# tensorflow/recommenders

Hardware: NVIDIA H100
Metric: queries/sec brute-force top-K (1Mx64 candidates) (higher is better)
Workload: dtype f32 (fp16 wgmma screening, fp32 accumulate + exact fp32 re-scoring)

## Files before the change

### include/tfrs_b200.h

```cpp
#ifndef TFRS_B200_H_
#define TFRS_B200_H_

#include <stddef.h>
#include <stdint.h>

#ifdef __cplusplus
extern "C" {
#endif

#define TFRS_B200_VERSION 102

enum {
  TFRS_OK = 0,
  TFRS_ERR_INVALID_ARG = -1,
  TFRS_ERR_UNSUPPORTED = -2,
  TFRS_ERR_CUDA = -3,
  TFRS_ERR_WORKSPACE_TOO_SMALL = -4,
  TFRS_ERR_NCCL = -5
};

enum { TFRS_I32 = 0, TFRS_I64 = 1 };

int tfrs_version(void);
const char* tfrs_last_error(void);
// ... 6 lines not shown
size_t tfrs_topk_scan_workspace_bytes(int64_t Q, int64_t N, int d, int k);
int tfrs_topk_scan_f32(const float* q, int64_t Q, const float* corpus, int64_t N, int d, int k,
                       int64_t index_offset, const float* state_scores, const int64_t* state_idx,
                       int state_k, float* out_scores, int64_t* out_idx, void* ws, size_t ws_bytes,
                       void* stream);

size_t tfrs_index_bytes(int64_t N, int d);
int tfrs_index_build(const float* corpus, int64_t N, int d, void* index_buf, size_t index_bytes,
                     void* stream);
size_t tfrs_topk_tc_workspace_bytes(int64_t Q, int64_t N, int d, int k);
int tfrs_topk_tc_f32(const float* q, int64_t Q, const float* corpus, const void* index_buf, int64_t N,
                     int d, int k, int64_t index_offset, float* out_scores, int64_t* out_idx, void* ws,
                     size_t ws_bytes, void* stream);

int tfrs_topk_tc_exclude_f32(const float* q, int64_t Q, const float* corpus, const void* index_buf, int64_t N, int d,
                             int k, int64_t index_offset, const int64_t* identifiers, const int64_t* exclusions,
                             int n_excl, float* out_scores, int64_t* out_idx, void* ws, size_t ws_bytes, void* stream);

int tfrs_topk_tc_count_f32(const float* q, int64_t Q, const float* corpus, const void* index_buf, int64_t N, int d,
                           int k, const float* positive_scores, int32_t* out_count, void* ws, size_t ws_bytes,
                           void* stream);

int tfrs_topk_exclude_rerank_f32(const float* scores, const int64_t* idx, int64_t Q, int k_fetched,
                                 const int64_t* identifiers, const int64_t* exclusions, int n_excl, int k_out,
                                 float* out_scores, int64_t* out_idx, void* stream);

int tfrs_count_above_f32(const float* scores, int64_t ld, int k, const float* positive_scores, int64_t Q,
                         int32_t* out_count, void* stream);

int tfrs_topk_hits_accumulate(const int32_t* count, const float* positive_scores, const float* sample_weight, int64_t Q,
                              const int32_t* ks, int n_ks, double* acc, void* stream);

int tfrs_topk_tc_layout(int64_t Q, int64_t N, int d, int k, int64_t* out10);

int tfrs_profile_enable(int on);
int tfrs_profile_read(float* stage_ms, int* calls);

int tfrs_topk_merge_strided(const float* scores, const int64_t* idx, int64_t list_stride_scores,
                            int64_t list_stride_idx, int n_lists, int64_t Q, int k_in, int k_out,
                            float* out_scores, int64_t* out_idx, void* stream);

int tfrs_topk_merge_sorted_strided(const float* scores, const int64_t* idx, int64_t list_stride_scores,
                                   int64_t list_stride_idx, int n_lists, int64_t Q, int k_in, int k_out,
                                   float* out_scores, int64_t* out_idx, void* stream);

typedef struct tfrs_comm* tfrs_comm_t;
int tfrs_comm_unique_id(void* out128);
int tfrs_comm_create(tfrs_comm_t* comm, int rank, int world, const void* unique_id128);
int tfrs_comm_destroy(tfrs_comm_t comm);
int tfrs_comm_enable_p2p(tfrs_comm_t comm, int64_t max_Q, int max_k);
int tfrs_comm_p2p_capacity(tfrs_comm_t comm, int64_t Q, int k);
int tfrs_comm_set_option(tfrs_comm_t comm, int option, int value);
int tfrs_comm_rank(tfrs_comm_t comm);
int tfrs_comm_world(tfrs_comm_t comm);
int tfrs_topk_allgather(tfrs_comm_t comm, const float* s, const int64_t* i, int64_t Q, int k, float* all_s,
                        int64_t* all_i, void* stream);
size_t tfrs_topk_sharded_workspace_bytes(int world, int64_t Q, int64_t N_local, int d, int k);
int tfrs_topk_sharded_layout(int world, int64_t Q, int64_t N_local, int d, int k, int64_t* out4);
int tfrs_topk_sharded_f32(tfrs_comm_t comm, const float* q, int64_t Q, const float* corpus_local, const void* index_buf,
                          int64_t N_local, int d, int k, int64_t index_offset, float* out_scores, int64_t* out_idx,
                          void* ws, size_t ws_bytes, void* stream);

int tfrs_sgemm_f32(int transA, int transB, int64_t M, int64_t N, int64_t K, const float* A, int64_t lda,
                   const float* B, int64_t ldb, float* C, int64_t ldc, int accumulate, void* stream);
int tfrs_rowwise_dot_f32(const float* a, const float* b, int64_t rows, int d, float* out, void* stream);

// ... 199 lines not shown
```

### recommenders_b200/_ffi.py

```python
from __future__ import annotations

import ctypes
import os
from typing import Optional

import torch

_HERE = os.path.dirname(os.path.abspath(__file__))
LIB_PATH = os.environ.get("TFRS_B200_LIB", os.path.join(_HERE, "libtfrs_b200.so"))

_lib: Optional[ctypes.CDLL] = None

I32, I64, BYTES = 0, 1, 2
c_p = ctypes.c_void_p
c_i = ctypes.c_int
c_l = ctypes.c_int64
c_f = ctypes.c_float
c_sz = ctypes.c_size_t

_SIGNATURES = {
    "tfrs_version": (c_i, []),
    "tfrs_last_error": (ctypes.c_char_p, []),
    "tfrs_launch_count": (c_l, []),
    "tfrs_gather_f32": (c_i, [c_p, c_p, c_p, c_i, c_p, c_i, c_l, c_p, c_l, c_p, c_p]),
    "tfrs_topk_scan_workspace_bytes": (c_sz, [c_l, c_l, c_i, c_i]),
    "tfrs_topk_scan_f32": (c_i, [c_p, c_l, c_p, c_l, c_i, c_i, c_l, c_p, c_p, c_i, c_p, c_p, c_p, c_sz, c_p]),
    "tfrs_index_bytes": (c_sz, [c_l, c_i]),
    "tfrs_index_build": (c_i, [c_p, c_l, c_i, c_p, c_sz, c_p]),
    "tfrs_topk_tc_workspace_bytes": (c_sz, [c_l, c_l, c_i, c_i]),
    "tfrs_topk_tc_f32": (c_i, [c_p, c_l, c_p, c_p, c_l, c_i, c_i, c_l, c_p, c_p, c_p, c_sz, c_p]),
    "tfrs_topk_tc_exclude_f32": (c_i, [c_p, c_l, c_p, c_p, c_l, c_i, c_i, c_l, c_p, c_p, c_i, c_p, c_p, c_p, c_sz, c_p]),
    "tfrs_topk_tc_count_f32": (c_i, [c_p, c_l, c_p, c_p, c_l, c_i, c_i, c_p, c_p, c_p, c_sz, c_p]),
    "tfrs_topk_exclude_rerank_f32": (c_i, [c_p, c_p, c_l, c_i, c_p, c_p, c_i, c_i, c_p, c_p, c_p]),
    "tfrs_count_above_f32": (c_i, [c_p, c_l, c_i, c_p, c_l, c_p, c_p]),
    "tfrs_topk_hits_accumulate": (c_i, [c_p, c_p, c_p, c_l, c_p, c_i, c_p, c_p]),
    "tfrs_topk_tc_layout": (c_i, [c_l, c_l, c_i, c_i, c_p]),
    "tfrs_dot_interaction_out_dim": (c_i, [c_i, c_i, c_i]),
    "tfrs_dot_interaction_fwd_f32": (c_i, [c_p, c_l, c_i, c_i, c_i, c_i, c_p, c_p]),
    "tfrs_dot_interaction_bwd_f32": (c_i, [c_p, c_p, c_l, c_i, c_i, c_i, c_i, c_p, c_p]),
    "tfrs_profile_enable": (c_i, [c_i]),
    "tfrs_profile_read": (c_i, [c_p, c_p]),
    "tfrs_topk_merge_strided": (c_i, [c_p, c_p, c_l, c_l, c_i, c_l, c_i, c_i, c_p, c_p, c_p]),
    "tfrs_topk_merge_sorted_strided": (c_i, [c_p, c_p, c_l, c_l, c_i, c_l, c_i, c_i, c_p, c_p, c_p]),
    "tfrs_comm_unique_id": (c_i, [c_p]),
    "tfrs_comm_create": (c_i, [c_p, c_i, c_i, c_p]),
    "tfrs_comm_destroy": (c_i, [c_p]),
    "tfrs_comm_enable_p2p": (c_i, [c_p, c_l, c_i]),
    "tfrs_comm_p2p_capacity": (c_i, [c_p, c_l, c_i]),
    "tfrs_comm_set_option": (c_i, [c_p, c_i, c_i]),
    "tfrs_comm_rank": (c_i, [c_p]),
    "tfrs_comm_world": (c_i, [c_p]),
    "tfrs_topk_allgather": (c_i, [c_p, c_p, c_p, c_l, c_i, c_p, c_p, c_p]),
    "tfrs_topk_sharded_workspace_bytes": (c_sz, [c_i, c_l, c_l, c_i, c_i]),
    "tfrs_topk_sharded_layout": (c_i, [c_i, c_l, c_l, c_i, c_i, c_p]),
    "tfrs_topk_sharded_f32": (c_i, [c_p, c_p, c_l, c_p, c_p, c_l, c_i, c_i, c_l, c_p, c_p, c_p, c_sz, c_p]),
    "tfrs_sgemm_f32": (c_i, [c_i, c_i, c_l, c_l, c_l, c_p, c_l, c_p, c_l, c_p, c_l, c_i, c_p]),
    "tfrs_rowwise_dot_f32": (c_i, [c_p, c_p, c_l, c_i, c_p, c_p]),
    "tfrs_inbatch_softmax_workspace_bytes": (c_sz, [c_l, c_l, c_i]),
    "tfrs_inbatch_softmax_fwd": (c_i, [c_p, c_p, c_l, c_l, c_i, c_f, c_p, c_p, c_p, c_p, c_sz, c_p]),
    "tfrs_inbatch_softmax_bwd": (c_i, [c_p, c_p, c_l, c_l, c_i, c_f, c_p, c_p, c_p, c_p, c_p, c_p, c_sz, c_p]),
    "tfrs_inbatch_softmax_tc_workspace_bytes": (c_sz, [c_l, c_l, c_i, c_i, c_i]),
    "tfrs_inbatch_softmax_tc_fwd": (c_i, [c_p, c_p, c_l, c_l, c_i, c_f, c_p, c_p, c_p, c_p, c_p, c_p, c_p, c_sz, c_p]),
    "tfrs_inbatch_softmax_tc_bwd_workspace_bytes": (c_sz, [c_l, c_l, c_i, c_i, c_i]),
    "tfrs_inbatch_softmax_tc_bwd": (c_i, [c_p, c_p, c_l, c_l, c_i, c_f, c_p, c_p, c_p, c_p, c_p, c_p, c_p, c_p, c_p, c_sz, c_p]),
    "tfrs_inbatch_softmax_maxsim_workspace_bytes": (c_sz, [c_l, c_i, c_l, c_i]),
    "tfrs_inbatch_softmax_maxsim_fwd": (c_i, [c_p, c_p, c_l, c_i, c_l, c_i, c_f, c_p, c_p, c_p, c_p, c_sz, c_p]),
    "tfrs_inbatch_softmax_maxsim_bwd": (c_i, [c_p, c_p, c_l, c_i, c_l, c_i, c_f, c_p, c_p, c_p, c_p, c_p, c_p, c_sz, c_p]),
    "tfrs_hardneg_loss_fwd": (c_i, [c_p, c_p, c_l, c_i, c_p, c_f, c_p, c_p, c_p, c_p]),
    "tfrs_hardneg_loss_bwd": (c_i, [c_p, c_p, c_l, c_l, c_i, c_p, c_i, c_p, c_p, c_p, c_p, c_p]),
# ... 140 lines not shown
```

### recommenders_b200/csrc/topk_tc.cu

```cuda
#include <cuda_fp16.h>
#include <math.h>
#include <stdlib.h>
#include <type_traits>
#include "rowselect.cuh"
#include "tc_ptx.cuh"

namespace tfrs {
namespace tc {

constexpr int TILE_N = 128;
constexpr int TILE_M = 128;
constexpr int QBLK = 256;
constexpr int KSLAB = 64;
constexpr int SLAB_BYTES = TILE_N * 128;
constexpr int HEADER_BYTES = 1024;
constexpr int THREADS = 512;
constexpr int CONSUMER_WARPS = 16;
constexpr int CAND_CAP = 2048;
constexpr int MAX_SAMPLE_STRIDE = 4;
constexpr int FIN_MAX_PARTS = 2 * 132;
constexpr int MAX_BINS = 1024;
constexpr int FP16_TARGET = 15;
constexpr float E_REL = 0.00108f;
constexpr float E_ACC = 0.00013f;
// ... 99 lines not shown
  const long long tile = row / TILE_N;
  if (lane < kb * 8) {
    const int slab = lane >> 3, cj = lane & 7;
    const int k0 = slab * KSLAB + cj * 8;
    __align__(16) __half v[8];
#pragma unroll
    for (int j = 0; j < 8; ++j) {
      const float f = (real && k0 + j < d) ? p[k0 + j] : 0.f;
      v[j] = __float2half_rn(ldexpf(f, e));
    }
    unsigned char* dst = qimg + tile * ((long long)kb * SLAB_BYTES) + (long long)slab * SLAB_BYTES + r * 128 + ((cj ^ (r & 7)) * 16);
    *reinterpret_cast<uint4*>(dst) = *reinterpret_cast<const uint4*>(v);
  }
}

enum { MODE_SAMPLE = 0, MODE_FILTER = 1 };

enum { FILTER_FULL = 0, FILTER_NO_EMIT = 1, FILTER_NO_EPILOGUE = 2 };
#if defined(TFRS_DEBUG_SWITCHES) && defined(TFRS_FILTER_ABLATION)
constexpr int FILTER_ABLATION = TFRS_FILTER_ABLATION;
#else
constexpr int FILTER_ABLATION = FILTER_FULL;
#endif

struct ScanParams {
  const unsigned char* qimg;
  const unsigned char* cimg;
  long long Q, N;
  int nqb, parts, n_seq, stride;
  long long n_tiles;
  float* binmax; int bins_ld;
  int group, bins_per_part;
  const float* thr;
  unsigned int* count;
  float* cand_s;
  unsigned int* cand_i;
  int cap_part;
};

template <int KB, int STAGES, int MODE>
__global__ void __launch_bounds__(THREADS, 1)
tc_scan_kernel(const ScanParams p) {
  extern __shared__ __align__(1024) unsigned char smem_raw[];
  unsigned char* smem = reinterpret_cast<unsigned char*>((reinterpret_cast<uintptr_t>(smem_raw) + 1023) & ~uintptr_t(1023));
  unsigned char* sA = smem;
  unsigned char* sB = smem + 2 * KB * SLAB_BYTES;
  uint64_t* bars = reinterpret_cast<uint64_t*>(sB + STAGES * KB * SLAB_BYTES);
  uint64_t* full = bars;
  uint64_t* empty = bars + STAGES;
  uint64_t* a_full = bars + 2 * STAGES;

  const int wg = threadIdx.x >> 7, warp = (threadIdx.x >> 5) & 3, lane = threadIdx.x & 31;
  const int qb = blockIdx.x % p.nqb, part = blockIdx.x / p.nqb;
  const int u_begin = (int)((long long)part * p.n_seq / p.parts);
  const int u_end = (int)((long long)(part + 1) * p.n_seq / p.parts);
  const int n_iter = u_end - u_begin;
  const bool issuer = threadIdx.x == 0;

  if (issuer) {
    for (int s = 0; s < STAGES; ++s) { mbar_init(&full[s], 1); mbar_init(&empty[s], CONSUMER_WARPS); }
    mbar_init(a_full, 1);
    asm volatile("fence.mbarrier_init.release.cluster;" ::: "memory");
  }
  __syncthreads();

  auto load_tile = [&](int it, int stage) {
    const long long tile = (long long)(u_begin + it) * p.stride;
    mbar_expect_tx(&full[stage], KB * SLAB_BYTES);
    if (MODE == MODE_FILTER)
      bulk_g2s_hint(sB + stage * KB * SLAB_BYTES, p.cimg + tile * ((long long)KB * SLAB_BYTES), KB * SLAB_BYTES, &full[stage],
                    l2_policy_evict_first());
    else
      bulk_g2s(sB + stage * KB * SLAB_BYTES, p.cimg + tile * ((long long)KB * SLAB_BYTES), KB * SLAB_BYTES, &full[stage]);
  };
  if (issuer) {
    mbar_expect_tx(a_full, 2 * KB * SLAB_BYTES);
    bulk_g2s(sA, p.qimg + (long long)qb * 2 * KB * SLAB_BYTES, 2 * KB * SLAB_BYTES, a_full);
    for (int it = 0; it < STAGES && it < n_iter; ++it) load_tile(it, it);
  }

  const long long row_a = (long long)qb * QBLK + wg * 64 + warp * 16 + (lane >> 2);
  const bool quad_leader = (lane & 3) == 0;
  float thr[2] = {INFINITY, INFINITY};
  if (MODE == MODE_FILTER) {
#pragma unroll
    for (int rr = 0; rr < 2; ++rr) if (row_a + 8 * rr < p.Q) thr[rr] = p.thr[row_a + 8 * rr];
  }
  const unsigned int cap = (unsigned int)p.cap_part;
  unsigned int cnt[4] = {0u, 0u, 0u, 0u}, ovf = 0u;
  unsigned int sink = 0u;
  long long seg_base[2];
#pragma unroll
  for (int rr = 0; rr < 2; ++rr) seg_base[rr] = ((row_a + 8 * rr) * p.parts + part) * 2 * (long long)cap;
  float binm[4] = {-INFINITY, -INFINITY, -INFINITY, -INFINITY};
  int in_group = 0, bin_out = 0;

  mbar_wait(a_full, 0);
  const uint32_t a0 = smem_u32(sA + (wg >> 1) * KB * SLAB_BYTES + (wg & 1) * 8192);
  uint32_t afrag[4][4];
  if (KB == 1) {
    const int r = warp * 16 + ((lane >> 3) & 1) * 8 + (lane & 7);
#pragma unroll
    for (int k4 = 0; k4 < 4; ++k4) ldmatrix_x4(afrag[k4], a0 + r * 128 + (((2 * k4 + (lane >> 4)) ^ (lane & 7)) * 16));
  }
  auto issue = [&](float (&acc)[32], int stage, int h) {
    wgmma_fence();
#pragma unroll
    for (int kb = 0; kb < KB; ++kb) {
      const uint64_t b_desc = make_smem_desc(smem_u32(sB + (stage * KB + kb) * SLAB_BYTES + h * 8192));
#pragma unroll
      for (int k4 = 0; k4 < 4; ++k4) {
        if (KB == 1)
          wgmma_m64n64_rs(acc, afrag[k4], b_desc + (uint64_t)(k4 * 2), (uint32_t)(k4 != 0));
        else
          wgmma_m64n64_ss(acc, make_smem_desc(a0 + kb * SLAB_BYTES) + (uint64_t)(k4 * 2), b_desc + (uint64_t)(k4 * 2),
                          (uint32_t)((kb | k4) != 0));
      }
    }
    wgmma_commit();
// ... 92 lines not shown
    __syncwarp();
    if (lane == 0) mbar_arrive(&empty[stage]);
    if (!LAST && issuer && it >= 1 && it - 1 + STAGES < n_iter) {
      mbar_wait(&empty[prev_stage], prev_phase);
      load_tile(it - 1 + STAGES, prev_stage);
    }
    prev_stage = stage; prev_phase = phase;
    stage = next_stage; phase = next_phase;
    epilogue(acc1, col0, it, std::integral_constant<int, 1>{});
    if (!LAST) {
      wgmma_wait<0>();
      acc_fence(acc0);
    }
  };
  if (n_iter > 0) {
    mbar_wait(&full[0], 0);
    issue(acc0, 0, 0);
    wgmma_wait<0>();
    acc_fence(acc0);
    for (int it = 0; it + 1 < n_iter; ++it) tile_step(it, std::false_type{});
    tile_step(n_iter - 1, std::true_type{});
  }
  if (MODE == MODE_SAMPLE) {
#pragma unroll
    for (int s = 0; s < 4; ++s) {
      const long long row = row_a + 8 * (s >> 1);
      if (quad_leader && row < p.Q)
        for (int b = bin_out; b < p.bins_per_part; ++b)
          p.binmax[row * p.bins_ld + (long long)part * p.bins_per_part * 2 + (s & 1) + 2 * b] = -INFINITY;
    }
  } else if (quad_leader) {
#pragma unroll
    for (int s = 0; s < 4; ++s)
      p.count[((row_a + 8 * (s >> 1)) * p.parts + part) * 2 + (s & 1)] =
          FILTER_ABLATION != FILTER_FULL ? sink : ((ovf >> s) & 1u) ? (cap + 1u) : cnt[s];
  }
}

__device__ __forceinline__ unsigned int f2key(float f) {
  unsigned int u = __float_as_uint(f);
  return (u & 0x80000000u) ? ~u : (u | 0x80000000u);
}
__device__ __forceinline__ float key2f(unsigned int k) {
  return __uint_as_float((k & 0x80000000u) ? (k & 0x7fffffffu) : ~k);
}
__device__ __forceinline__ unsigned long long rank_key(float s, unsigned int idx) {
  const unsigned int lo = (0xFFFFFFFEu - 2u * idx) | (__float_as_uint(s) == 0x80000000u ? 1u : 0u);
  return ((unsigned long long)f2key(s + 0.0f) << 32) | lo;
}
__device__ __forceinline__ float rank_key_score(unsigned long long e) {
  return __uint_as_float(__float_as_uint(key2f((unsigned int)(e >> 32))) | ((unsigned int)e << 31));
}
__device__ __forceinline__ unsigned int rank_key_index(unsigned long long e) { return 0x7FFFFFFFu - ((unsigned int)e >> 1); }
__device__ __forceinline__ int warp_incl_scan(int v, int lane) {
#pragma unroll
  for (int o = 1; o < 32; o <<= 1) { const int t = __shfl_up_sync(0xffffffffu, v, o); if (lane >= o) v += t; }
  return v;
}

template <int KPL>
__device__ __forceinline__ unsigned int warp_kth_largest_regs(const unsigned int (&key)[KPL], int k, unsigned int prefix = 0, int top_bit = 31) {
  for (int bit = top_bit; bit >= 0; --bit) {
    const unsigned int cand = prefix | (1u << bit);
    int c = 0;
#pragma unroll
    for (int j = 0; j < KPL; ++j) c += (key[j] >= cand) ? 1 : 0;
    c = __reduce_add_sync(0xffffffffu, c);
    if (c >= k) prefix = cand;
  }
  return prefix;
}
__device__ __forceinline__ unsigned int warp_kth_largest_smem(const unsigned int* keys, int n, int k, int lane, unsigned int prefix, int top_bit) {
  for (int bit = top_bit; bit >= 0; --bit) {
    const unsigned int cand = prefix | (1u << bit);
    int c = 0;
    for (int t = lane; t < n; t += 32) c += (keys[t] >= cand) ? 1 : 0;
    c = __reduce_add_sync(0xffffffffu, c);
    if (c >= k) prefix = cand;
  }
  return prefix;
}

template <int KPL>
__global__ void __launch_bounds__(256)
tc_threshold_kernel(const float* __restrict__ binmax, int bins_ld, int n_bins, int k, const float* __restrict__ margin,
                    float* __restrict__ thr, unsigned int* __restrict__ overflow, long long Q) {
  const int lane = threadIdx.x & 31;
  const long long row = ((long long)blockIdx.x * 256 + threadIdx.x) >> 5;
  if (row >= Q) return;
  const float* src = binmax + row * bins_ld;
  unsigned int key[KPL];
#pragma unroll
  for (int j = 0; j < KPL; ++j) { const int i = j * 32 + lane; key[j] = i < n_bins ? f2key(__ldg(src + i)) : 0u; }
  const unsigned int kth = warp_kth_largest_regs<KPL>(key, k);
  if (lane == 0) { thr[row] = key2f(kth) - margin[row]; overflow[row] = 0; }
}

enum { FIN_TOPK = 0, FIN_EXCLUDE = 1, FIN_COUNT = 2 };
constexpr int FW_WARPS = 4;

struct FinParams {
  const float* q; const float* corpus; int d; int k; long long index_offset; long long N; long long Q;
  const unsigned int* count; const float* cand_s; const unsigned int* cand_i; int segs; int cap_part;
  const float* cut; const float* thr; unsigned int* overflow;
  int cap_keys, cap_band;
  unsigned int* band_idx; int* band_n;
  int allow_short;
  float* out_s; long long* out_i;
  const long long* identifiers; const long long* exclusions; int n_excl; int k_out;
  const float* pos; const int* qexp; const IndexHeader* hdr; int* out_count;
};

__device__ __forceinline__ float exact_score(const float* __restrict__ qs, const float* __restrict__ c, int d) {
  float acc = 0.f;
  if ((d & 31) == 0) {
    for (int kk = 0; kk < d; kk += 32) {
      float4 cv[8];
#pragma unroll
      for (int u = 0; u < 8; ++u) cv[u] = __ldg(reinterpret_cast<const float4*>(c + kk) + u);
#pragma unroll
      for (int u = 0; u < 8; ++u) {
        acc = fmaf(qs[kk + 4 * u], cv[u].x, acc); acc = fmaf(qs[kk + 4 * u + 1], cv[u].y, acc);
        acc = fmaf(qs[kk + 4 * u + 2], cv[u].z, acc); acc = fmaf(qs[kk + 4 * u + 3], cv[u].w, acc);
      }
    }
  } else if ((d & 3) == 0) {
    for (int kk = 0; kk < d; kk += 4) {
      const float4 cv = __ldg(reinterpret_cast<const float4*>(c + kk));
      acc = fmaf(qs[kk], cv.x, acc); acc = fmaf(qs[kk + 1], cv.y, acc);
      acc = fmaf(qs[kk + 2], cv.z, acc); acc = fmaf(qs[kk + 3], cv.w, acc);
    }
  } else {
    for (int kk = 0; kk < d; ++kk) acc = fmaf(qs[kk], __ldg(c + kk), acc);
  }
  return acc;
}

// ... 39 lines not shown
    for (int j = 0; j < kf; ++j) rank += (akey[j] > mine) ? 1 : 0;
    if (rank < p.k_out) {
      const unsigned long long e = srt[t];
      p.out_s[row * p.k_out + rank] = rank_key_score(e);
      p.out_i[row * p.k_out + rank] = (long long)rank_key_index(e) + p.index_offset;
    }
  }
}

__host__ __device__ inline size_t sel_warp_bytes(int cap_keys, int segs) {
  return (size_t)cap_keys * 4 + (size_t)cap_keys * 2 + (size_t)((segs + 1 + 3) & ~3) * 4;
}
constexpr int SEL_WARPS = 8;

__device__ __forceinline__ bool load_record(const FinParams& p, long long row, const int* soff, int rec, int total_rec,
                                            unsigned int& ix0, float (&sc)[8]) {
  if (rec >= total_rec) return false;
  int lo = 0, hi = p.segs;
  while (hi - lo > 1) { const int mid = (lo + hi) >> 1; if (soff[mid] <= rec) lo = mid; else hi = mid; }
  const long long at = (row * p.segs + lo) * p.cap_part + (rec - soff[lo]);
  ix0 = __ldg(p.cand_i + at);
  const float4 s0 = __ldg(reinterpret_cast<const float4*>(p.cand_s + at * 8));
  const float4 s1 = __ldg(reinterpret_cast<const float4*>(p.cand_s + at * 8) + 1);
  sc[0] = s0.x; sc[1] = s0.y; sc[2] = s0.z; sc[3] = s0.w; sc[4] = s1.x; sc[5] = s1.y; sc[6] = s1.z; sc[7] = s1.w;
  return true;
}

template <int MODE>
__global__ void __launch_bounds__(SEL_WARPS * 32)
tc_select_kernel(const FinParams p) {
  extern __shared__ __align__(16) unsigned char fsm[];
  const int warp = threadIdx.x >> 5, lane = threadIdx.x & 31;
  const long long row = (long long)blockIdx.x * SEL_WARPS + warp;
  if (row >= p.Q) return;
  unsigned char* base = fsm + (size_t)warp * sel_warp_bytes(p.cap_keys, p.segs);
  unsigned int* keys = reinterpret_cast<unsigned int*>(base);
  unsigned short* loc = reinterpret_cast<unsigned short*>(keys + p.cap_keys);
  int* soff = reinterpret_cast<int*>(loc + p.cap_keys);
  const unsigned int n32 = (unsigned int)p.N;
  unsigned int* band = p.band_idx + row * p.cap_band;

  int carry = 0; bool bad = false;
  for (int s0 = 0; s0 < p.segs; s0 += 32) {
    const int s = s0 + lane;
    int c = 0;
    if (s < p.segs) {
      const unsigned int cc = __ldg(p.count + row * p.segs + s);
      if (cc > (unsigned int)p.cap_part) bad = true; else c = (int)cc;
    }
    const int inc = warp_incl_scan(c, lane);
    if (s < p.segs) soff[s + 1] = carry + inc;
    carry += __shfl_sync(0xffffffffu, inc, 31);
  }
  if (lane == 0) soff[0] = 0;
  if (__any_sync(0xffffffffu, bad)) {
    if (lane == 0) { p.overflow[row] = 1; p.band_n[row] = 0; }
    return;
  }
  __syncwarp();
  const int total_rec = soff[p.segs];
  const float thr_row = p.thr[row];
  if (MODE != FIN_COUNT && total_rec >= 8192) {
    if (lane == 0) { p.overflow[row] = 1; p.band_n[row] = 0; }
    return;
  }

  if (MODE == FIN_COUNT) {
// ... 29 lines not shown
      else { p.out_count[row] = definite; p.band_n[row] = m; p.overflow[row] = 0; }
    }
    return;
  }

  int n = 0;
  unsigned int kmax = 0u, kmin = 0xFFFFFFFFu;
  for (int rb = 0; rb < total_rec; rb += 32) {
    float sc[8]; unsigned int ix0 = 0, keep = 0; int cnt = 0;
    if (load_record(p, row, soff, rb + lane, total_rec, ix0, sc)) {
#pragma unroll
      for (int j = 0; j < 8; ++j) {
        const bool kp = sc[j] >= thr_row && ix0 + j < n32;
        keep |= kp ? (1u << j) : 0u; cnt += kp ? 1 : 0;
      }
    }
    const int incl = warp_incl_scan(cnt, lane);
    const int tot = __shfl_sync(0xffffffffu, incl, 31);
    if (n + tot <= p.cap_keys) {
      int at_pos = n + incl - cnt;
#pragma unroll
      for (int j = 0; j < 8; ++j) {
        if (keep & (1u << j)) {
          const unsigned int key = f2key(sc[j] + 0.0f);
          kmax = max(kmax, key); kmin = min(kmin, key);
          keys[at_pos] = key;
          loc[at_pos] = (unsigned short)(((rb + lane) << 3) | j);
          ++at_pos;
        }
      }
    }
    n += tot;
  }
  if (n > p.cap_keys || (n < p.k && !p.allow_short)) { if (lane == 0) { p.overflow[row] = 1; p.band_n[row] = 0; } return; }
  __syncwarp();
  if (n < p.k) {
    const bool fits = n <= p.cap_band;
    for (int t = lane; t < n && fits; t += 32) {
      const unsigned int l = loc[t];
      const int rec = (int)(l >> 3);
      int lo = 0, hi = p.segs;
      while (hi - lo > 1) { const int mid = (lo + hi) >> 1; if (soff[mid] <= rec) lo = mid; else hi = mid; }
      band[t] = __ldg(p.cand_i + (row * p.segs + lo) * p.cap_part + (rec - soff[lo])) + (l & 7u);
    }
    if (lane == 0) { p.overflow[row] = fits ? 0u : 1u; p.band_n[row] = fits ? n : 0; }
    return;
  }
  kmax = __reduce_max_sync(0xffffffffu, kmax); kmin = __reduce_min_sync(0xffffffffu, kmin);
  unsigned int tau_key;
  {
    const unsigned int diff = kmax ^ kmin;
    const int top = diff ? (31 - __clz(diff)) : -1;
    const unsigned int prefix0 = top >= 31 ? 0u : (top < 0 ? kmax : (kmax & ~((2u << top) - 1u)));
    if (n <= 512) {
      unsigned int kr[16];
#pragma unroll
      for (int j = 0; j < 16; ++j) { const int t = j * 32 + lane; kr[j] = t < n ? keys[t] : 0u; }
      tau_key = warp_kth_largest_regs<16>(kr, p.k, prefix0, top);
    } else if (n <= 1024) {
      unsigned int kr[32];
#pragma unroll
      for (int j = 0; j < 32; ++j) { const int t = j * 32 + lane; kr[j] = t < n ? keys[t] : 0u; }
      tau_key = warp_kth_largest_regs<32>(kr, p.k, prefix0, top);
    } else {
      tau_key = warp_kth_largest_smem(keys, n, p.k, lane, prefix0, top);
    }
  }
  const float lim = key2f(tau_key) - p.cut[row];
  if (!p.allow_short && (!(lim >= thr_row) || !(lim > -INFINITY))) { if (lane == 0) { p.overflow[row] = 1; p.band_n[row] = 0; } return; }
  const unsigned int lim_key = f2key(lim + 0.0f);
  const unsigned int lt_mask = (1u << lane) - 1u;
  int m = 0;
  for (int tb = 0; tb < n; tb += 32) {
    const int t = tb + lane;
    const bool kp = t < n && keys[t] >= lim_key;
    const unsigned int vote = __ballot_sync(0xffffffffu, kp);
    if (kp) {
      const int at_pos = m + __popc(vote & lt_mask);
      if (at_pos < p.cap_band) {
        const unsigned int l = loc[t];
        const int rec = (int)(l >> 3);
        int lo = 0, hi = p.segs;
        while (hi - lo > 1) { const int mid = (lo + hi) >> 1; if (soff[mid] <= rec) lo = mid; else hi = mid; }
        band[at_pos] = __ldg(p.cand_i + (row * p.segs + lo) * p.cap_part + (rec - soff[lo])) + (l & 7u);
      }
    }
    m += __popc(vote);
  }
  if (lane == 0) {
    if (m > p.cap_band) { p.overflow[row] = 1; p.band_n[row] = 0; }
    else { p.overflow[row] = 0; p.band_n[row] = m; }
  }
}

constexpr int RS_BLOCK = 128;
template <int MODE>
__global__ void __launch_bounds__(RS_BLOCK)
tc_rescore_kernel(const FinParams p) {
  extern __shared__ __align__(16) unsigned char rsm[];
  unsigned long long* sk = reinterpret_cast<unsigned long long*>(rsm);
  float* qs = reinterpret_cast<float*>(sk + p.cap_band);
  unsigned long long* srt = reinterpret_cast<unsigned long long*>(qs + ((p.d + 3) & ~3));
// ... 124 lines not shown
  for (long long t = threadIdx.x; t < N; t += 256) {
    const float* cr = corpus + t * d;
    float acc = 0.f;
    for (int kk = 0; kk < d; ++kk) acc = fmaf(qs[kk], __ldg(cr + kk), acc);
    c += (acc + 0.0f > ps) ? 1 : 0;
  }
  c = __reduce_add_sync(0xffffffffu, c);
  if ((threadIdx.x & 31) == 0) atomicAdd(&total, c);
  __syncthreads();
  if (threadIdx.x == 0) out_count[row] = total < k ? total : k;
}

struct Prof {
  bool on = false;
  static constexpr int MAXC = 512, STAGES_ = 4;
  cudaEvent_t ev[MAXC][STAGES_ + 1];
  int created = 0, calls = 0;
};
static Prof g_prof;
static void prof_mark(cudaStream_t st, int stage) {
  if (!g_prof.on || g_prof.calls >= Prof::MAXC) return;
  int c = g_prof.calls;
  while (g_prof.created <= c) {
    for (int s = 0; s <= Prof::STAGES_; ++s) cudaEventCreate(&g_prof.ev[g_prof.created][s]);
    ++g_prof.created;
  }
  cudaEventRecord(g_prof.ev[c][stage], st);
  if (stage == Prof::STAGES_) ++g_prof.calls;
}

struct Plan {
  int kb, stages; long long n_tiles; int nqb; long long Qp;
  int stride, n_sample, group, bins_per_part, n_bins, bins_ld, parts_sample, parts_full, cap_part, cap_keys, cap_band;
  size_t smem;
  size_t o_qimg, o_margin, o_cut, o_thr, o_qexp, o_count, o_ovf, o_binmax, o_cand, o_tmp, o_band, o_bandn, total;
};

static bool make_plan(long long Q, long long N, int d, int k, Plan& pl) {
  if (d <= 0 || d > 128 || Q <= 0 || N <= 0 || k <= 0) return false;
  pl.kb = (d + KSLAB - 1) / KSLAB;
  pl.stages = pl.kb == 1 ? 6 : 4;
  pl.n_tiles = ceil_div(N, TILE_N);
  pl.nqb = (int)ceil_div(Q, QBLK);
  pl.Qp = (long long)pl.nqb * QBLK;
  if (k > 256 || N >= (1ll << 31)) return false;
  const long long full_tiles = N / TILE_N;
  if (full_tiles < 1) return false;
  pl.stride = MAX_SAMPLE_STRIDE;
#ifdef TFRS_DEBUG_SWITCHES
  { static int ov = getenv("TFRS_TC_SAMPLE_STRIDE") ? atoi(getenv("TFRS_TC_SAMPLE_STRIDE")) : 0; if (ov >= 1 && ov <= 16) pl.stride = ov; }
#endif
  while (pl.stride > 1 && 2 * ceil_div(full_tiles, pl.stride) < 4ll * k) pl.stride >>= 1;
  pl.n_sample = (int)ceil_div(full_tiles, pl.stride);
  if (2ll * pl.n_sample < 4ll * k) return false;
  const int sms = sm_count();
  int parts = sms / pl.nqb; if (parts < 1) parts = 1; if (parts > FIN_MAX_PARTS / 2) parts = FIN_MAX_PARTS / 2;
  pl.parts_sample = parts < pl.n_sample ? parts : pl.n_sample;
  pl.parts_full = (long long)parts < pl.n_tiles ? parts : (int)pl.n_tiles;
  {
    const int iters_max = (int)ceil_div(pl.n_sample, pl.parts_sample);
    const int target = 4 * k > 512 ? 4 * k : 512;
    int g = 1;
    while ((long long)pl.parts_sample * ceil_div(iters_max, g) * 2 > target && g < iters_max) ++g;
    pl.group = g;
    pl.bins_per_part = (int)ceil_div(iters_max, g);
    pl.n_bins = pl.parts_sample * pl.bins_per_part * 2;
    if (pl.n_bins > MAX_BINS || pl.n_bins < 2 * k) return false;
    pl.bins_ld = (pl.n_bins + 31) / 32 * 32;
  }
  {
    const double lambda = (double)k * pl.stride / (pl.parts_full * 2.0);
    const double want = 2.0 * lambda + 12.0 * sqrt(lambda) + 8.0;
    int p2 = 32; while (p2 < want && p2 < 512) p2 <<= 1;
    pl.cap_part = p2;
    int ck = 1024; while (ck < 1.6 * 1.3 * k * pl.stride && ck < 4096) ck <<= 1;
    pl.cap_keys = ck;
    pl.cap_band = ck / 2;
  }
  pl.smem = (size_t)(2 + pl.stages) * pl.kb * SLAB_BYTES + 1024  + 256 ;
  size_t o = 0;
  auto take = [&](size_t bytes) { size_t r = o; o += align_up(bytes, 1024); return r; };
  pl.o_qimg = take((size_t)pl.nqb * 2 * pl.kb * SLAB_BYTES);
  pl.o_margin = take((size_t)pl.Qp * 4);
  pl.o_cut = take((size_t)pl.Qp * 4);
  pl.o_thr = take((size_t)pl.Qp * 4);
  pl.o_qexp = take((size_t)pl.Qp * 4);
  pl.o_count = take((size_t)pl.Qp * pl.parts_full * 2 * 4);
  pl.o_ovf = take((size_t)pl.Qp * 4);
  pl.o_binmax = take((size_t)pl.Qp * pl.bins_ld * 4);
  pl.o_cand = take((size_t)pl.Qp * pl.parts_full * 2 * pl.cap_part * (8 * 4 + 4));
  pl.o_tmp = take((size_t)Q * k * 12);
  pl.o_band = take((size_t)pl.Qp * pl.cap_band * 4);
  pl.o_bandn = take((size_t)pl.Qp * 4);
  pl.total = o;
  return true;
}

template <int KB, int STAGES>
static int launch_scans(const Plan& pl, ScanParams sp, cudaStream_t st, int mode) {
  auto ks = tc_scan_kernel<KB, STAGES, MODE_SAMPLE>;
  auto kf = tc_scan_kernel<KB, STAGES, MODE_FILTER>;
  TFRS_DYN_SMEM(ks, (int)pl.smem);
  TFRS_DYN_SMEM(kf, (int)pl.smem);
  if (mode == MODE_SAMPLE) {
    sp.parts = pl.parts_sample; sp.n_seq = pl.n_sample; sp.stride = pl.stride;
    ks<<<(unsigned)(pl.nqb * sp.parts), THREADS, pl.smem, st>>>(sp);
  } else {
    sp.parts = pl.parts_full; sp.n_seq = (int)pl.n_tiles; sp.stride = 1;
    kf<<<(unsigned)(pl.nqb * sp.parts), THREADS, pl.smem, st>>>(sp);
  }
  TFRS_LAUNCH_CHECK();
  return TFRS_OK;
}

static int launch_scan_mode(const Plan& pl, const ScanParams& sp, cudaStream_t st, int mode) {
  if (pl.kb == 1) return launch_scans<1, 6>(pl, sp, st, mode);
  return launch_scans<2, 4>(pl, sp, st, mode);
}

template <int MODE>
static int launch_finalize(FinParams fp, cudaStream_t st) {
  auto ksel = tc_select_kernel<MODE>;
  auto krs = tc_rescore_kernel<MODE>;
  TFRS_DYN_SMEM(ksel, (int)(SEL_WARPS * sel_warp_bytes(4096, FIN_MAX_PARTS)));
  ksel<<<(unsigned)ceil_div(fp.Q, SEL_WARPS), SEL_WARPS * 32, SEL_WARPS * sel_warp_bytes(fp.cap_keys, fp.segs), st>>>(fp);
  TFRS_LAUNCH_CHECK();
  const size_t rs_smem = (size_t)fp.cap_band * 8 + (size_t)((fp.d + 3) & ~3) * 4 + (MODE == FIN_EXCLUDE ? (size_t)fp.k * 16 : 0);
  TFRS_DYN_SMEM(krs, 64 * 1024);
  krs<<<(unsigned)fp.Q, RS_BLOCK, rs_smem, st>>>(fp);
  TFRS_LAUNCH_CHECK();
  return TFRS_OK;
}

struct Call {
  int mode;
  const float* q; long long Q; const float* corpus; const void* index_buf; long long N; int d; int k; long long index_offset;
  void* ws; size_t ws_bytes; cudaStream_t st;
  float* out_s; long long* out_i;
  const long long* identifiers; const long long* exclusions; int n_excl; int k_out;
  const float* pos; int* out_count;
  ThrHook hook; void* hook_ctx; int allow_short;
};

static int run_call(const Call& c) {
  Plan pl;
  if (!make_plan(c.Q, c.N, c.d, c.k, pl)) {
    set_error("topk_tc: shape (Q=%lld N=%lld d=%d k=%d) is outside the tensor-core path; use tfrs_topk_scan_f32",
              c.Q, c.N, c.d, c.k);
    return TFRS_ERR_UNSUPPORTED;
  }
  if (!c.ws || c.ws_bytes < pl.total + 16) { set_error("topk_tc: workspace too small (%zu < %zu)", c.ws_bytes, pl.total + 16); return TFRS_ERR_WORKSPACE_TOO_SMALL; }
  cudaStream_t st = c.st;
  unsigned char* w = (unsigned char*)(((uintptr_t)c.ws + 15) & ~(uintptr_t)15);
  unsigned char* qimg = w + pl.o_qimg;
  float* margin = (float*)(w + pl.o_margin);
  float* cut = (float*)(w + pl.o_cut);
  float* thr = (float*)(w + pl.o_thr);
  int* qexp = (int*)(w + pl.o_qexp);
  unsigned int* count = (unsigned int*)(w + pl.o_count);
  unsigned int* ovf = (unsigned int*)(w + pl.o_ovf);
  float* binmax = (float*)(w + pl.o_binmax);
  float* cand_s = (float*)(w + pl.o_cand);
  unsigned int* cand_i = (unsigned int*)(w + pl.o_cand + (size_t)pl.Qp * pl.parts_full * 2 * pl.cap_part * 32);
  float* tmp_s = (float*)(w + pl.o_tmp);
  long long* tmp_i = (long long*)(w + pl.o_tmp + align_up((size_t)c.Q * c.k * 4, 8));
  const IndexHeader* hdr = (const IndexHeader*)c.index_buf;
  const unsigned char* cimg = (const unsigned char*)c.index_buf + HEADER_BYTES;

  prof_mark(st, 0);
  tc_qprep_kernel<<<(unsigned)ceil_div(pl.Qp * 32, 256), 256, 0, st>>>(c.q, c.Q, pl.Qp, c.d, pl.kb, hdr, qimg, margin, cut, qexp);
  TFRS_LAUNCH_CHECK();
  ScanParams sp{};
  sp.qimg = qimg; sp.cimg = cimg; sp.Q = c.Q; sp.N = c.N; sp.nqb = pl.nqb; sp.n_tiles = pl.n_tiles;
  sp.binmax = binmax; sp.bins_ld = pl.bins_ld; sp.group = pl.group; sp.bins_per_part = pl.bins_per_part;
  sp.thr = thr; sp.count = count; sp.cand_s = cand_s; sp.cand_i = cand_i; sp.cap_part = pl.cap_part;
  prof_mark(st, 1);
  int rc = launch_scan_mode(pl, sp, st, MODE_SAMPLE);
  if (rc) return rc;
  if (pl.n_bins <= 512)
    tc_threshold_kernel<16><<<(unsigned)ceil_div(c.Q * 32, 256), 256, 0, st>>>(binmax, pl.bins_ld, pl.n_bins, c.k, margin, thr, ovf, c.Q);
  else
    tc_threshold_kernel<32><<<(unsigned)ceil_div(c.Q * 32, 256), 256, 0, st>>>(binmax, pl.bins_ld, pl.n_bins, c.k, margin, thr, ovf, c.Q);
  TFRS_LAUNCH_CHECK();
  if (c.hook) {
    rc = c.hook(c.hook_ctx, thr, margin, cut, qexp, &hdr->st.exp, c.Q, st);
    if (rc) return rc;
  }
  prof_mark(st, 2);
  rc = launch_scan_mode(pl, sp, st, MODE_FILTER);
  if (rc) return rc;
  prof_mark(st, 3);
  if (FILTER_ABLATION != FILTER_FULL) { prof_mark(st, 4); return TFRS_OK; }
  FinParams fp{};
  fp.q = c.q; fp.corpus = c.corpus; fp.d = c.d; fp.k = c.k; fp.index_offset = c.index_offset; fp.N = c.N; fp.Q = c.Q;
  fp.count = count; fp.cand_s = cand_s; fp.cand_i = cand_i; fp.segs = pl.parts_full * 2; fp.cap_part = pl.cap_part;
  fp.cut = cut; fp.thr = thr; fp.overflow = ovf; fp.out_s = c.out_s; fp.out_i = c.out_i;
  fp.cap_keys = pl.cap_keys; fp.cap_band = pl.cap_band; fp.allow_short = c.allow_short;
  fp.band_idx = (unsigned int*)(w + pl.o_band); fp.band_n = (int*)(w + pl.o_bandn);
  fp.identifiers = c.identifiers; fp.exclusions = c.exclusions; fp.n_excl = c.n_excl; fp.k_out = c.k_out;
  fp.pos = c.pos; fp.qexp = qexp; fp.hdr = hdr; fp.out_count = c.out_count;
  if (c.mode == FIN_TOPK) rc = launch_finalize<FIN_TOPK>(fp, st);
  else if (c.mode == FIN_EXCLUDE) rc = launch_finalize<FIN_EXCLUDE>(fp, st);
  else rc = launch_finalize<FIN_COUNT>(fp, st);
  if (rc) return rc;
  if (c.mode == FIN_COUNT) {
    tc_count_fallback_kernel<<<(unsigned)c.Q, 256, 0, st>>>(c.q, c.corpus, c.N, c.d, c.k, c.pos, ovf, c.out_count);
    TFRS_LAUNCH_CHECK();
  } else {
    FallbackProvider prov{c.q, c.corpus, c.N, c.d, c.index_offset, ovf, nullptr};
    int cap = rowselect_cap(c.k);
    TFRS_DYN_SMEM(row_topk_kernel<FallbackProvider>, 64 * 1024);
    float* fs = c.mode == FIN_TOPK ? c.out_s : tmp_s;
    long long* fi = c.mode == FIN_TOPK ? c.out_i : tmp_i;
    row_topk_kernel<FallbackProvider><<<(unsigned)c.Q, RS_THREADS, rowselect_smem(cap, (size_t)c.d * 4), st>>>(prov, c.k, cap, fs, fi, c.k);
    TFRS_LAUNCH_CHECK();
    if (c.mode == FIN_EXCLUDE) {
      tc_exclude_fallback_kernel<<<(unsigned)ceil_div(c.Q, FW_WARPS), FW_WARPS * 32, (size_t)FW_WARPS * 2 * c.k * 8, st>>>(fp, tmp_s, tmp_i, ovf);
      TFRS_LAUNCH_CHECK();
    }
  }
  prof_mark(st, 4);
  return TFRS_OK;
}

}
}

using namespace tfrs;
using namespace tfrs::tc;

extern "C" size_t tfrs_index_bytes(int64_t N, int d) {
  if (N <= 0 || d <= 0 || d > 128) return 0;
  int kb = (d + KSLAB - 1) / KSLAB;
  return (size_t)HEADER_BYTES + (size_t)ceil_div(N, TILE_N) * kb * SLAB_BYTES;
}

// ... 57 lines not shown
                                        int n_excl, float* out_scores, int64_t* out_idx, void* ws, size_t ws_bytes, void* stream) {
  TFRS_CHECK_ARG(q && corpus && index_buf && out_scores && out_idx && exclusions && n_excl > 0, "topk_tc_exclude: bad argument");
  TFRS_CHECK_ARG((long long)k + n_excl <= N, "input must have at least k columns. Had %lld, needed %d", (long long)N, k + n_excl);
  Call c{};
  c.mode = FIN_EXCLUDE; c.q = q; c.Q = Q; c.corpus = corpus; c.index_buf = index_buf; c.N = N; c.d = d; c.k = k + n_excl;
  c.index_offset = index_offset; c.ws = ws; c.ws_bytes = ws_bytes; c.st = (cudaStream_t)stream;
  c.out_s = out_scores; c.out_i = (long long*)out_idx;
  c.identifiers = (const long long*)identifiers; c.exclusions = (const long long*)exclusions; c.n_excl = n_excl; c.k_out = k;
  return run_call(c);
}

extern "C" int tfrs_topk_tc_count_f32(const float* q, int64_t Q, const float* corpus, const void* index_buf, int64_t N, int d,
                                      int k, const float* positive_scores, int32_t* out_count, void* ws, size_t ws_bytes,
                                      void* stream) {
  TFRS_CHECK_ARG(q && corpus && index_buf && positive_scores && out_count, "topk_tc_count: NULL pointer");
  TFRS_CHECK_ARG(k <= N, "input must have at least k columns. Had %lld, needed %d", (long long)N, k);
  Call c{};
  c.mode = FIN_COUNT; c.q = q; c.Q = Q; c.corpus = corpus; c.index_buf = index_buf; c.N = N; c.d = d; c.k = k;
  c.ws = ws; c.ws_bytes = ws_bytes; c.st = (cudaStream_t)stream;
  c.pos = positive_scores; c.out_count = out_count;
  return run_call(c);
}

extern "C" int tfrs_topk_tc_layout(int64_t Q, int64_t N, int d, int k, int64_t* out10) {
  TFRS_CHECK_ARG(out10, "topk_tc_layout: NULL pointer");
  Plan pl;
  if (!make_plan(Q, N, d, k, pl)) { set_error("topk_tc_layout: unsupported shape"); return TFRS_ERR_UNSUPPORTED; }
  out10[0] = (int64_t)pl.o_count; out10[1] = (int64_t)pl.o_ovf; out10[2] = (int64_t)pl.o_thr; out10[3] = (int64_t)pl.o_cand;
  out10[4] = pl.parts_full * 2; out10[5] = pl.cap_part; out10[6] = pl.Qp; out10[7] = (int64_t)pl.o_cut;
  out10[8] = pl.n_bins; out10[9] = (int64_t)pl.o_qexp;
  return TFRS_OK;
}

extern "C" int tfrs_profile_enable(int on) {
  g_prof.on = on != 0;
  g_prof.calls = 0;
  return TFRS_OK;
}

extern "C" int tfrs_profile_read(float* stage_ms, int* calls) {
  TFRS_CHECK_ARG(stage_ms && calls, "profile_read: NULL pointer");
  TFRS_CUDA(cudaDeviceSynchronize());
  for (int s = 0; s < 4; ++s) stage_ms[s] = 0.f;
  for (int c = 0; c < g_prof.calls; ++c)
    for (int s = 0; s < 4; ++s) {
      float ms = 0.f;
      TFRS_CUDA(cudaEventElapsedTime(&ms, g_prof.ev[c][s], g_prof.ev[c][s + 1]));
      stage_ms[s] += ms;
    }
  *calls = g_prof.calls;
  return TFRS_OK;
}
```

Before: 2.744 million.

## Use tighter probabilistic filter threshold with selective per-query rescan fallback

The threshold kernel now computes two thresholds from sampled bin maxima: a conservative one at rank k, and a tighter one at a lower rank chosen from a binomial tail bound on the sample stride. The filter scan uses the tighter threshold, so fewer candidates are admitted and the selection stage does less work. Queries whose filtered set comes up short are marked for retry. Those blocks rerun the filter scan with the safe threshold, and all other blocks exit early. The cost is an extra scan launch and a second select launch on every call, even when no query needs a retry.

```diff
diff --git a/include/tfrs_b200.h b/include/tfrs_b200.h
--- a/include/tfrs_b200.h
+++ b/include/tfrs_b200.h
@@ -62,6 +62,8 @@
                               const int32_t* ks, int n_ks, double* acc, void* stream);
 
 int tfrs_topk_tc_layout(int64_t Q, int64_t N, int d, int k, int64_t* out10);
+
+int tfrs_topk_tc_retry_layout(int64_t Q, int64_t N, int d, int k, int64_t* out4);
 
 int tfrs_profile_enable(int on);
 int tfrs_profile_read(float* stage_ms, int* calls);
diff --git a/recommenders_b200/_ffi.py b/recommenders_b200/_ffi.py
--- a/recommenders_b200/_ffi.py
+++ b/recommenders_b200/_ffi.py
@@ -35,6 +35,7 @@
     "tfrs_count_above_f32": (c_i, [c_p, c_l, c_i, c_p, c_l, c_p, c_p]),
     "tfrs_topk_hits_accumulate": (c_i, [c_p, c_p, c_p, c_l, c_p, c_i, c_p, c_p]),
     "tfrs_topk_tc_layout": (c_i, [c_l, c_l, c_i, c_i, c_p]),
+    "tfrs_topk_tc_retry_layout": (c_i, [c_l, c_l, c_i, c_i, c_p]),
     "tfrs_dot_interaction_out_dim": (c_i, [c_i, c_i, c_i]),
     "tfrs_dot_interaction_fwd_f32": (c_i, [c_p, c_l, c_i, c_i, c_i, c_i, c_p, c_p]),
     "tfrs_dot_interaction_bwd_f32": (c_i, [c_p, c_p, c_l, c_i, c_i, c_i, c_i, c_p, c_p]),
diff --git a/recommenders_b200/csrc/topk_tc.cu b/recommenders_b200/csrc/topk_tc.cu
--- a/recommenders_b200/csrc/topk_tc.cu
+++ b/recommenders_b200/csrc/topk_tc.cu
@@ -155,6 +155,7 @@
   float* binmax; int bins_ld;
   int group, bins_per_part;
   const float* thr;
+  const unsigned int* retry;
   unsigned int* count;
   float* cand_s;
   unsigned int* cand_i;
@@ -179,6 +180,10 @@
   const int u_end = (int)((long long)(part + 1) * p.n_seq / p.parts);
   const int n_iter = u_end - u_begin;
   const bool issuer = threadIdx.x == 0;
+  auto rescanned = [&](long long row) { return p.retry == nullptr || (row < p.Q && p.retry[row] != 0u); };
+  if (MODE == MODE_FILTER && p.retry != nullptr &&
+      !__syncthreads_or(threadIdx.x < QBLK && rescanned((long long)qb * QBLK + threadIdx.x)))
+    return;
 
   if (issuer) {
     for (int s = 0; s < STAGES; ++s) { mbar_init(&full[s], 1); mbar_init(&empty[s], CONSUMER_WARPS); }
@@ -207,7 +212,7 @@
   float thr[2] = {INFINITY, INFINITY};
   if (MODE == MODE_FILTER) {
 #pragma unroll
-    for (int rr = 0; rr < 2; ++rr) if (row_a + 8 * rr < p.Q) thr[rr] = p.thr[row_a + 8 * rr];
+    for (int rr = 0; rr < 2; ++rr) if (row_a + 8 * rr < p.Q) thr[rr] = rescanned(row_a + 8 * rr) ? p.thr[row_a + 8 * rr] : NAN;
   }
   const unsigned int cap = (unsigned int)p.cap_part;
   unsigned int cnt[4] = {0u, 0u, 0u, 0u}, ovf = 0u;
@@ -366,8 +371,9 @@
   } else if (quad_leader) {
 #pragma unroll
     for (int s = 0; s < 4; ++s)
-      p.count[((row_a + 8 * (s >> 1)) * p.parts + part) * 2 + (s & 1)] =
-          FILTER_ABLATION != FILTER_FULL ? sink : ((ovf >> s) & 1u) ? (cap + 1u) : cnt[s];
+      if (rescanned(row_a + 8 * (s >> 1)))
+        p.count[((row_a + 8 * (s >> 1)) * p.parts + part) * 2 + (s & 1)] =
+            FILTER_ABLATION != FILTER_FULL ? sink : ((ovf >> s) & 1u) ? (cap + 1u) : cnt[s];
   }
 }
 
@@ -417,8 +423,9 @@
 
 template <int KPL>
 __global__ void __launch_bounds__(256)
-tc_threshold_kernel(const float* __restrict__ binmax, int bins_ld, int n_bins, int k, const float* __restrict__ margin,
-                    float* __restrict__ thr, unsigned int* __restrict__ overflow, long long Q) {
+tc_threshold_kernel(const float* __restrict__ binmax, int bins_ld, int n_bins, int k, int k_filter, const float* __restrict__ margin,
+                    float* __restrict__ thr, float* __restrict__ thr_safe, unsigned int* __restrict__ overflow,
+                    unsigned int* __restrict__ retry, long long Q) {
   const int lane = threadIdx.x & 31;
   const long long row = ((long long)blockIdx.x * 256 + threadIdx.x) >> 5;
   if (row >= Q) return;
@@ -426,8 +433,9 @@
   unsigned int key[KPL];
 #pragma unroll
   for (int j = 0; j < KPL; ++j) { const int i = j * 32 + lane; key[j] = i < n_bins ? f2key(__ldg(src + i)) : 0u; }
-  const unsigned int kth = warp_kth_largest_regs<KPL>(key, k);
-  if (lane == 0) { thr[row] = key2f(kth) - margin[row]; overflow[row] = 0; }
+  const float safe = key2f(warp_kth_largest_regs<KPL>(key, k)) - margin[row];
+  const float filter = k_filter < k ? key2f(warp_kth_largest_regs<KPL>(key, k_filter)) - margin[row] : safe;
+  if (lane == 0) { thr[row] = filter; thr_safe[row] = safe; overflow[row] = 0; retry[row] = 0; }
 }
 
 enum { FIN_TOPK = 0, FIN_EXCLUDE = 1, FIN_COUNT = 2 };
@@ -436,7 +444,8 @@
 struct FinParams {
   const float* q; const float* corpus; int d; int k; long long index_offset; long long N; long long Q;
   const unsigned int* count; const float* cand_s; const unsigned int* cand_i; int segs; int cap_part;
-  const float* cut; const float* thr; unsigned int* overflow;
+  const float* cut; float* thr; const float* thr_safe; unsigned int* overflow;
+  unsigned int* retry; int retry_pass;
   int cap_keys, cap_band;
   unsigned int* band_idx; int* band_n;
   int allow_short;
@@ -542,7 +551,7 @@
   extern __shared__ __align__(16) unsigned char fsm[];
   const int warp = threadIdx.x >> 5, lane = threadIdx.x & 31;
   const long long row = (long long)blockIdx.x * SEL_WARPS + warp;
-  if (row >= p.Q) return;
+  if (row >= p.Q || (p.retry_pass && p.retry[row] == 0u)) return;
   unsigned char* base = fsm + (size_t)warp * sel_warp_bytes(p.cap_keys, p.segs);
   unsigned int* keys = reinterpret_cast<unsigned int*>(base);
   unsigned short* loc = reinterpret_cast<unsigned short*>(keys + p.cap_keys);
@@ -638,7 +647,15 @@
     }
     n += tot;
   }
-  if (n > p.cap_keys || (n < p.k && !p.allow_short)) { if (lane == 0) { p.overflow[row] = 1; p.band_n[row] = 0; } return; }
+  auto miss = [&]() {
+    if (lane == 0) {
+      const float safe = p.thr_safe[row];
+      if (thr_row > safe) { p.retry[row] = 1; p.thr[row] = safe; } else p.overflow[row] = 1;
+      p.band_n[row] = 0;
+    }
+  };
+  if (n > p.cap_keys) { if (lane == 0) { p.overflow[row] = 1; p.band_n[row] = 0; } return; }
+  if (n < p.k && !p.allow_short) { miss(); return; }
   __syncwarp();
   if (n < p.k) {
     const bool fits = n <= p.cap_band;
@@ -673,7 +690,7 @@
     }
   }
   const float lim = key2f(tau_key) - p.cut[row];
-  if (!p.allow_short && (!(lim >= thr_row) || !(lim > -INFINITY))) { if (lane == 0) { p.overflow[row] = 1; p.band_n[row] = 0; } return; }
+  if (!p.allow_short && (!(lim >= thr_row) || !(lim > -INFINITY))) { miss(); return; }
   const unsigned int lim_key = f2key(lim + 0.0f);
   const unsigned int lt_mask = (1u << lane) - 1u;
   int m = 0;
@@ -864,9 +881,23 @@
 struct Plan {
   int kb, stages; long long n_tiles; int nqb; long long Qp;
   int stride, n_sample, group, bins_per_part, n_bins, bins_ld, parts_sample, parts_full, cap_part, cap_keys, cap_band;
+  int k_filter;
   size_t smem;
-  size_t o_qimg, o_margin, o_cut, o_thr, o_qexp, o_count, o_ovf, o_binmax, o_cand, o_tmp, o_band, o_bandn, total;
+  size_t o_qimg, o_margin, o_cut, o_thr, o_qexp, o_count, o_ovf, o_binmax, o_cand, o_tmp, o_band, o_bandn, o_thr_safe, o_retry,
+      total;
 };
+
+static int filter_bin_rank(int k, int stride) {
+  if (stride <= 1 || k <= 1) return k;
+  const int n = k - 1;
+  const double p = 1.0 / stride;
+  double tail = 0.0;
+  for (int r = n; r >= 1; --r) {
+    tail += exp(lgamma(n + 1.0) - lgamma(r + 1.0) - lgamma(n - r + 1.0) + r * log(p) + (n - r) * log1p(-p));
+    if (tail > 1e-9) return r + 1;
+  }
+  return 1;
+}
 
 static bool make_plan(long long Q, long long N, int d, int k, Plan& pl) {
   if (d <= 0 || d > 128 || Q <= 0 || N <= 0 || k <= 0) return false;
@@ -883,6 +914,7 @@
   { static int ov = getenv("TFRS_TC_SAMPLE_STRIDE") ? atoi(getenv("TFRS_TC_SAMPLE_STRIDE")) : 0; if (ov >= 1 && ov <= 16) pl.stride = ov; }
 #endif
   while (pl.stride > 1 && 2 * ceil_div(full_tiles, pl.stride) < 4ll * k) pl.stride >>= 1;
+  pl.k_filter = filter_bin_rank(k, pl.stride);
   pl.n_sample = (int)ceil_div(full_tiles, pl.stride);
   if (2ll * pl.n_sample < 4ll * k) return false;
   const int sms = sm_count();
@@ -924,6 +956,8 @@
   pl.o_tmp = take((size_t)Q * k * 12);
   pl.o_band = take((size_t)pl.Qp * pl.cap_band * 4);
   pl.o_bandn = take((size_t)pl.Qp * 4);
+  pl.o_thr_safe = take((size_t)pl.Qp * 4);
+  pl.o_retry = take((size_t)pl.Qp * 4);
   pl.total = o;
   return true;
 }
@@ -951,12 +985,20 @@
 }
 
 template <int MODE>
-static int launch_finalize(FinParams fp, cudaStream_t st) {
+static int launch_finalize(FinParams fp, const Plan& pl, ScanParams sp, bool retry, cudaStream_t st) {
   auto ksel = tc_select_kernel<MODE>;
   auto krs = tc_rescore_kernel<MODE>;
   TFRS_DYN_SMEM(ksel, (int)(SEL_WARPS * sel_warp_bytes(4096, FIN_MAX_PARTS)));
   ksel<<<(unsigned)ceil_div(fp.Q, SEL_WARPS), SEL_WARPS * 32, SEL_WARPS * sel_warp_bytes(fp.cap_keys, fp.segs), st>>>(fp);
   TFRS_LAUNCH_CHECK();
+  if (retry) {
+    sp.retry = fp.retry;
+    const int rc = launch_scan_mode(pl, sp, st, MODE_FILTER);
+    if (rc) return rc;
+    fp.retry_pass = 1;
+    ksel<<<(unsigned)ceil_div(fp.Q, SEL_WARPS), SEL_WARPS * 32, SEL_WARPS * sel_warp_bytes(fp.cap_keys, fp.segs), st>>>(fp);
+    TFRS_LAUNCH_CHECK();
+  }
   const size_t rs_smem = (size_t)fp.cap_band * 8 + (size_t)((fp.d + 3) & ~3) * 4 + (MODE == FIN_EXCLUDE ? (size_t)fp.k * 16 : 0);
   TFRS_DYN_SMEM(krs, 64 * 1024);
   krs<<<(unsigned)fp.Q, RS_BLOCK, rs_smem, st>>>(fp);
@@ -996,8 +1038,11 @@
   unsigned int* cand_i = (unsigned int*)(w + pl.o_cand + (size_t)pl.Qp * pl.parts_full * 2 * pl.cap_part * 32);
   float* tmp_s = (float*)(w + pl.o_tmp);
   long long* tmp_i = (long long*)(w + pl.o_tmp + align_up((size_t)c.Q * c.k * 4, 8));
+  float* thr_safe = (float*)(w + pl.o_thr_safe);
+  unsigned int* retry = (unsigned int*)(w + pl.o_retry);
   const IndexHeader* hdr = (const IndexHeader*)c.index_buf;
   const unsigned char* cimg = (const unsigned char*)c.index_buf + HEADER_BYTES;
+  const int k_filter = (c.mode == FIN_COUNT || c.hook) ? c.k : pl.k_filter;
 
   prof_mark(st, 0);
   tc_qprep_kernel<<<(unsigned)ceil_div(pl.Qp * 32, 256), 256, 0, st>>>(c.q, c.Q, pl.Qp, c.d, pl.kb, hdr, qimg, margin, cut, qexp);
@@ -1010,9 +1055,11 @@
   int rc = launch_scan_mode(pl, sp, st, MODE_SAMPLE);
   if (rc) return rc;
   if (pl.n_bins <= 512)
-    tc_threshold_kernel<16><<<(unsigned)ceil_div(c.Q * 32, 256), 256, 0, st>>>(binmax, pl.bins_ld, pl.n_bins, c.k, margin, thr, ovf, c.Q);
+    tc_threshold_kernel<16><<<(unsigned)ceil_div(c.Q * 32, 256), 256, 0, st>>>(binmax, pl.bins_ld, pl.n_bins, c.k, k_filter, margin,
+                                                                                 thr, thr_safe, ovf, retry, c.Q);
   else
-    tc_threshold_kernel<32><<<(unsigned)ceil_div(c.Q * 32, 256), 256, 0, st>>>(binmax, pl.bins_ld, pl.n_bins, c.k, margin, thr, ovf, c.Q);
+    tc_threshold_kernel<32><<<(unsigned)ceil_div(c.Q * 32, 256), 256, 0, st>>>(binmax, pl.bins_ld, pl.n_bins, c.k, k_filter, margin,
+                                                                                 thr, thr_safe, ovf, retry, c.Q);
   TFRS_LAUNCH_CHECK();
   if (c.hook) {
     rc = c.hook(c.hook_ctx, thr, margin, cut, qexp, &hdr->st.exp, c.Q, st);
@@ -1026,14 +1073,15 @@
   FinParams fp{};
   fp.q = c.q; fp.corpus = c.corpus; fp.d = c.d; fp.k = c.k; fp.index_offset = c.index_offset; fp.N = c.N; fp.Q = c.Q;
   fp.count = count; fp.cand_s = cand_s; fp.cand_i = cand_i; fp.segs = pl.parts_full * 2; fp.cap_part = pl.cap_part;
-  fp.cut = cut; fp.thr = thr; fp.overflow = ovf; fp.out_s = c.out_s; fp.out_i = c.out_i;
+  fp.cut = cut; fp.thr = thr; fp.thr_safe = thr_safe; fp.overflow = ovf; fp.retry = retry; fp.out_s = c.out_s; fp.out_i = c.out_i;
   fp.cap_keys = pl.cap_keys; fp.cap_band = pl.cap_band; fp.allow_short = c.allow_short;
   fp.band_idx = (unsigned int*)(w + pl.o_band); fp.band_n = (int*)(w + pl.o_bandn);
   fp.identifiers = c.identifiers; fp.exclusions = c.exclusions; fp.n_excl = c.n_excl; fp.k_out = c.k_out;
   fp.pos = c.pos; fp.qexp = qexp; fp.hdr = hdr; fp.out_count = c.out_count;
-  if (c.mode == FIN_TOPK) rc = launch_finalize<FIN_TOPK>(fp, st);
-  else if (c.mode == FIN_EXCLUDE) rc = launch_finalize<FIN_EXCLUDE>(fp, st);
-  else rc = launch_finalize<FIN_COUNT>(fp, st);
+  const bool may_retry = k_filter < c.k;
+  if (c.mode == FIN_TOPK) rc = launch_finalize<FIN_TOPK>(fp, pl, sp, may_retry, st);
+  else if (c.mode == FIN_EXCLUDE) rc = launch_finalize<FIN_EXCLUDE>(fp, pl, sp, may_retry, st);
+  else rc = launch_finalize<FIN_COUNT>(fp, pl, sp, false, st);
   if (rc) return rc;
   if (c.mode == FIN_COUNT) {
     tc_count_fallback_kernel<<<(unsigned)c.Q, 256, 0, st>>>(c.q, c.corpus, c.N, c.d, c.k, c.pos, ovf, c.out_count);
@@ -1157,6 +1205,14 @@
   return TFRS_OK;
 }
 
+extern "C" int tfrs_topk_tc_retry_layout(int64_t Q, int64_t N, int d, int k, int64_t* out4) {
+  TFRS_CHECK_ARG(out4, "topk_tc_retry_layout: NULL pointer");
+  Plan pl;
+  if (!make_plan(Q, N, d, k, pl)) { set_error("topk_tc_retry_layout: unsupported shape"); return TFRS_ERR_UNSUPPORTED; }
+  out4[0] = (int64_t)pl.o_thr_safe; out4[1] = (int64_t)pl.o_retry; out4[2] = pl.k_filter; out4[3] = pl.stride;
+  return TFRS_OK;
+}
+
 extern "C" int tfrs_profile_enable(int on) {
   g_prof.on = on != 0;
   g_prof.calls = 0;
```

After: 3.077 million, median of 6. 1.12x the previous value.
